# keikoproj/active-monitor

Measured on AMD Instinct MI355X. Metric: sustained_healthcheck_cycles_per_sec, higher is better.
Workload: dtype n/a; 1 GPU; model=healthcheck-controller, global_batch=1000, seq_len=0, parallelism=shard1x8w, crs_per_rank=1000, workers_per_rank=8, max_concurrent_crs=1000, cr_mix=49% repeatAfterSec, 30% cron, 20% failing-with-remedy, apiserver=http-subprocess-127.0.0.1

## Files before the change

active_monitor_amd/kube/http.py:

```python
from __future__ import annotations

import asyncio
import json
import logging
import re
import ssl
import time
from collections import deque
from typing import Any, AsyncIterator, Dict, List, Optional, Tuple
from urllib.parse import urlencode, urlsplit

import aiohttp

from ..utils import wirecodec
from .auth import Credential, CredentialSource
from .errors import (
    AlreadyExistsError,
    ApiError,
    BadRequestError,
    ConflictError,
    InvalidError,
    NotFoundError,
    UnauthorizedError,
)
# ... 233 lines not shown
    def __init__(self, qps: float, burst: int):
        self.qps = qps
        self.burst = float(burst)
        self.tokens = float(burst)
        self.last = time.monotonic()
        self._lock = asyncio.Lock()

    async def acquire(self) -> None:
        if self.qps <= 0:
            return
        async with self._lock:
            now = time.monotonic()
            self.tokens = min(self.burst, self.tokens + (now - self.last) * self.qps)
            self.last = now
            if self.tokens >= 1.0:
                self.tokens -= 1.0
                return
            wait = (1.0 - self.tokens) / self.qps
            self.tokens = 0.0
            await asyncio.sleep(wait)
            self.last = time.monotonic()


class _ConnPool:

    def __init__(self, host: str, port: int, max_conns: int = 32):
        self.host = host
        self.port = port
        self.max_conns = max_conns
        self._free: List[Tuple[asyncio.StreamReader, asyncio.StreamWriter]] = []
        self._count = 0
        self._waiters: "deque[asyncio.Future]" = deque()
        self._closed = False

    async def _acquire(self):
        while True:
            while self._free:
                reader, writer = self._free.pop()
                if writer.is_closing():
                    self._count -= 1
                    continue
                return reader, writer
            if self._count < self.max_conns:
                self._count += 1
                try:
                    return await asyncio.open_connection(self.host, self.port)
                except Exception:
                    self._count -= 1
                    raise
            fut = asyncio.get_running_loop().create_future()
            self._waiters.append(fut)
            await fut

    def _release(self, conn, reusable: bool) -> None:
        if reusable and not self._closed and not conn[1].is_closing():
            self._free.append(conn)
        else:
            self._count -= 1
            try:
                conn[1].close()
            except Exception:
                pass
        while self._waiters:
            fut = self._waiters.popleft()
            if not fut.done():
                fut.set_result(None)
                break

    async def request(self, method: str, target: str, headers: str,
                      body: Optional[bytes]) -> Tuple[int, bytes]:
        head = (
            f"{method} {target} HTTP/1.1\r\nHost: {self.host}:{self.port}\r\n"
            f"{headers}Content-Length: {len(body) if body else 0}\r\n\r\n"
        ).encode("latin-1")
        return await self._roundtrip(head + body if body else head)

    async def request_json(self, method: str, target: str, headers: str,
                           obj: Optional[Obj]) -> Tuple[int, bytes]:
        prefix = (
            f"{method} {target} HTTP/1.1\r\nHost: {self.host}:{self.port}\r\n"
            f"{headers}"
        ).encode("latin-1")
        return await self._roundtrip(wirecodec.frame(prefix, obj))

    async def _roundtrip(self, data: bytes) -> Tuple[int, bytes]:
        conn = await self._acquire()
        reader, writer = conn
        ok = False
        try:
            writer.write(data)
            await writer.drain()

            try:
                head = await reader.readuntil(b"\r\n\r\n")
            except asyncio.IncompleteReadError as e:
                if not e.partial:
                    raise ConnectionResetError("server closed connection") from None
                raise
            status, content_length, chunked, keep_alive = (
                wirecodec.parse_response_head(head)
            )
            if chunked:
                chunks = []
                while True:
                    size_line = await reader.readline()
                    size = int(size_line.strip().split(b";")[0], 16)
                    if size == 0:
                        await reader.readline()
                        break
                    chunks.append(await reader.readexactly(size))
                    await reader.readexactly(2)
                payload = b"".join(chunks)
            else:
                payload = await reader.readexactly(content_length) if content_length else b""
            ok = keep_alive
            return status, payload
        finally:
            self._release(conn, ok)

    def close(self) -> None:
        self._closed = True
        for _, writer in self._free:
            try:
                writer.close()
            except Exception:
                pass
        self._free.clear()
        while self._waiters:
            fut = self._waiters.popleft()
            if not fut.done():
                fut.set_exception(ConnectionError("connection pool closed"))


class HttpClient:
    def __init__(
        self,
        base_url: str,
        token: Optional[str] = None,
        verify: bool = True,
        ca_cert: Optional[str] = None,
        registry: Registry = DEFAULT_REGISTRY,
        qps: float = 20.0,
        burst: int = 30,
        credentials: Optional[CredentialSource] = None,
    ):
        self.base_url = base_url.rstrip("/")
        self.token = token
# ... 224 lines not shown
```

active_monitor_amd/kube/server.py:

```python
from __future__ import annotations

import asyncio
import hmac
import logging
from typing import List, Optional, Set, Tuple

from ..utils import wirecodec
from ..utils.wirecodec import EXPECT_CONTINUE, WANT_TABLE
from .errors import (
    ApiError,
    BadRequestError,
    ExpiredError,
    InvalidError,
    NotFoundError,
    UnauthorizedError,
)
from .memory import (
    MemoryApiServer,
    fields_match,
    labels_match,
    object_rv,
    parse_field_selector,
    parse_label_selector,
)
from .registry import WF_API_VERSION, WF_KIND

log = logging.getLogger("active_monitor_amd.kube.server")

_REASONS = {
    200: "OK", 201: "Created", 400: "Bad Request", 401: "Unauthorized",
    404: "Not Found",
# ... 75 lines not shown
        out = []
        for byte in path.encode("utf-8", "surrogatepass"):
            if byte in (0x22, 0x5C):
                out.append("\\" + chr(byte))
            elif 0x20 <= byte <= 0x7E and byte != 0x25:
                out.append(chr(byte))
            else:
                out.append(f"%{byte:02X}")
        return "".join(out)

    def prefix(self, status: int) -> bytes:
        lines = "".join(
            f'Warning: 299 - "unknown field \\"{self._header_text(p)}\\""\r\n'
            for p in self.paths
        )
        return _json_prefix(status) + lines.encode("ascii")


_OPEN_PATHS = frozenset({
    "/healthz", "/livez", "/readyz", "/version", "/version/",
})


class ApiServerFrontend:
    def __init__(self, server: MemoryApiServer, host: str = "127.0.0.1", port: int = 0,
                 accepted_tokens: Optional[Set[str]] = None, logs=None):
        self.server = server
        self.logs = logs
        self.host = host
        self.port = port
        self.accepted_tokens = accepted_tokens
        self.unauthorized_count = 0
        self._srv: Optional[asyncio.AbstractServer] = None
        self._live_subs: list = []

    @property
    def url(self) -> str:
        return f"http://{self.host}:{self.port}"

    async def start(self) -> None:
        self._srv = await asyncio.start_server(self._handle_conn, self.host, self.port)
        if self.port == 0:
            self.port = self._srv.sockets[0].getsockname()[1]

    async def stop(self) -> None:
        self.kick_watches()
        if self._srv is not None:
            self._srv.close()
            try:
                await asyncio.wait_for(self._srv.wait_closed(), 2.0)
            except asyncio.TimeoutError:
                pass

    def kick_watches(self) -> None:
        for sub in list(self._live_subs):
            sub.close()


    def _authorized(self, path: str, authorization: bytes) -> bool:
        if path in _OPEN_PATHS:
            return True
        ok = False
        scheme, _, presented = authorization.partition(b" ")
        if scheme.lower() == b"bearer":
            presented = presented.strip()
            for tok in list(self.accepted_tokens or ()):
                if hmac.compare_digest(presented, tok.encode("utf-8")):
                    ok = True
        if not ok:
            self.unauthorized_count += 1
        return ok

    @staticmethod
    def _unauthorized_response() -> bytes:
        return wirecodec.frame(
            _UNAUTHORIZED_PREFIX, _status_body(UnauthorizedError("Unauthorized"))
        )


    async def _handle_conn(self, reader: asyncio.StreamReader,
                           writer: asyncio.StreamWriter) -> None:
        try:
            while True:
                head = await reader.readuntil(b"\r\n\r\n")
                parsed = wirecodec.parse_request_head(head)
                if parsed is None:
                    return
                (method, path, query, content_length, content_type, flags,
                 authorization) = parsed
                if flags & EXPECT_CONTINUE:
                    writer.write(b"HTTP/1.1 100 Continue\r\n\r\n")
                    await writer.drain()
                body = await reader.readexactly(content_length) if content_length else b""

                if (self.accepted_tokens is not None
                        and not self._authorized(path, authorization)):
                    writer.write(self._unauthorized_response())
                    await writer.drain()
                    continue
                if query.get("watch") in ("true", "1"):
                    await self._serve_watch(writer, path, query)
                    return
                if path.endswith("/log") and self._is_log_route(path):
                    if await self._serve_log(writer, method, path, query):
                        return
                    continue
                status, obj = self._serve_unary(method, path, query, body,
                                                content_type)
                if (flags & WANT_TABLE and method == "GET" and status == 200
                        and isinstance(obj, dict)):
                    obj = self._to_table(obj)
                if type(obj) is dict or not isinstance(obj, (_Warned, str)):
                    writer.write(wirecodec.frame(_json_prefix(status), obj))
                elif isinstance(obj, _Warned):
                    writer.write(wirecodec.frame(obj.prefix(status), obj.obj))
                else:
                    payload = obj.encode()
                    writer.write(
                        (
                            f"HTTP/1.1 {status} {_REASONS.get(status, 'OK')}\r\n"
                            f"Content-Type: text/plain\r\n"
                            f"Content-Length: {len(payload)}\r\n\r\n"
                        ).encode("latin-1") + payload
                    )
                await writer.drain()
        except (ConnectionError, asyncio.IncompleteReadError,
                asyncio.LimitOverrunError, asyncio.CancelledError):
            pass
        except Exception:
            log.exception("frontend connection handler failed")
        finally:
            try:
                writer.close()
            except Exception:
                pass


    def _serve_unary(self, method: str, path: str, query: dict,
                     body: bytes, content_type: str = "") -> Tuple[int, Optional[dict]]:
        if path in ("/api", "/api/"):
            return 200, {"kind": "APIVersions", "versions": ["v1"]}
        if path in ("/apis", "/apis/"):
            return 200, self._discovery_apis()
        if path in ("/version", "/version/"):
            from .. import __version__

            return 200, {
                "major": "1", "minor": "33",
                "gitVersion": f"v1.33.0-active-monitor-amd+{__version__}",
            }
        if path in ("/healthz", "/readyz", "/livez"):
            return 200, "ok"
        route = _route(path)
        if route is None:
            return _failure(ApiError(f"the server could not find {path}"), 404)
        if not route[2]:
            return 200, self._resource_list(route[0])
        return self._dispatch(method, route, query, body, content_type)
# ... 195 lines not shown
                    "kind": "PartialObjectMetadata",
                    "apiVersion": "meta.k8s.io/v1",
                    "metadata": it.get("metadata", {}),
                },
            })
        return {
            "kind": "Table",
            "apiVersion": "meta.k8s.io/v1",
            "metadata": meta,
            "columnDefinitions": defs,
            "rows": rows,
        }


    def _is_log_route(self, path: str) -> bool:
        route = _route(path)
        if route is None or route[4] != "log" or route[0] != WF_API_VERSION:
            return False
        try:
            return self.server.registry.by_plural(route[0], route[2]).kind == WF_KIND
        except KeyError:
            return False

    async def _serve_log(self, writer: asyncio.StreamWriter, method: str,
                         path: str, query: dict) -> bool:
        _, namespace, _, name, _ = _route(path)
        try:
            if method != "GET":
                raise _MethodNotAllowed(f"unsupported method {method}")
            numbers = {}
            for key in ("tailLines", "limitBytes"):
                if query.get(key) is not None:
                    try:
                        numbers[key] = int(query[key])
                    except ValueError:
                        raise BadRequestError(
                            f"{key} must be an integer, not {query[key]!r}")
            self.server.get(WF_API_VERSION, WF_KIND, namespace, name)
            if self.logs is None:
                raise NotFoundError(
                    f"workflow {namespace}/{name} has no logs: this server "
                    "keeps no workflow logs")
            if not self.logs.has_run(namespace, name):
                raise NotFoundError(
                    f"workflow {namespace}/{name} has no logs: it was not run "
                    "by the local executor, or its logs were dropped for the "
                    "total size cap")
# ... 19 lines not shown
            return False
        self._live_subs.append(stream)
        try:
            writer.write(
                b"HTTP/1.1 200 OK\r\nContent-Type: text/plain\r\n"
                b"Transfer-Encoding: chunked\r\nConnection: close\r\n\r\n"
            )
            await writer.drain()
            async for chunk in stream:
                writer.write(b"%x\r\n%s\r\n" % (len(chunk), chunk))
                await writer.drain()
            writer.write(b"0\r\n\r\n")
            await writer.drain()
        except (ConnectionError, asyncio.CancelledError):
            pass
        finally:
            await stream.aclose()
            if stream in self._live_subs:
                self._live_subs.remove(stream)
        return True


    @staticmethod
    async def _refuse_watch(writer: asyncio.StreamWriter, err: ApiError,
                            status: int) -> None:
        status, body = _failure(err, status)
        writer.write(wirecodec.frame(_json_prefix(status), body))
        await writer.drain()

    async def _serve_watch(self, writer: asyncio.StreamWriter, path: str,
                           query: dict) -> None:
        route = _route(path)
        if route is None:
            return await self._refuse_watch(
                writer, ApiError(f"the server could not find {path}"), 404)
        api_version, namespace, plural = route[:3]
        namespace = namespace or None
        try:
            kind = self.server.registry.by_plural(api_version, plural).kind
        except KeyError:
            tail = [seg for seg in path.split("/") if seg][api_version.count("/") + 2:]
            return await self._refuse_watch(
                writer, ApiError("unknown resource " + "/".join(tail)), 404)

        rv_param = query.get("resourceVersion")
        selector: dict = {}
        fields: List[tuple] = []
        try:
            selector = parse_label_selector(query.get("labelSelector"))
        except ApiError:
            pass
        try:
            fields = parse_field_selector(query.get("fieldSelector"))
# ... 67 lines not shown
```

active_monitor_amd/utils/wirecodec.py:

```python
from __future__ import annotations

import json
import os
from typing import Any, Dict, Iterator, Optional, Tuple
from urllib.parse import parse_qsl, unquote, urlsplit

EXPECT_CONTINUE = 1
WANT_TABLE = 2

RequestHead = Tuple[str, str, Dict[str, str], int, str, int, bytes]
ResponseHead = Tuple[int, int, bool, bool]



def _py_dumpb(obj: Any) -> bytes:
    return json.dumps(obj, separators=(",", ":")).encode()


def _py_frame(prefix: bytes, obj: Any) -> bytes:
    payload = json.dumps(obj, separators=(",", ":")).encode() if obj is not None else b""
    return prefix + (
        f"Content-Length: {len(payload)}\r\n\r\n"
    ).encode("latin-1") + payload

# ... 55 lines not shown

def _py_parse_response_head(head: bytes) -> ResponseHead:
    lines = _head_lines(head)
    status_line = next(lines, b"")
    if not status_line:
        raise ConnectionResetError("server closed connection")
    status = int(status_line.split(b" ", 2)[1])
    content_length = 0
    chunked = False
    keep_alive = True
    for line in lines:
        if line in (b"\r\n", b"\n", b""):
            break
        lower = line.lower()
        if lower.startswith(b"content-length:"):
            content_length = int(line.split(b":", 1)[1])
        elif lower.startswith(b"transfer-encoding:") and b"chunked" in lower:
            chunked = True
        elif lower.startswith(b"connection:") and b"close" in lower:
            keep_alive = False
    return status, content_length, chunked, keep_alive



try:
    from active_monitor_amd import _amcore

    _json_dumpb = _amcore.json_dumpb
    _json_frame = _amcore.json_frame
    _json_loadb = _amcore.json_loadb
    _parse_request_head = _amcore.parse_request_head
    _parse_response_head = _amcore.parse_response_head
    HAVE_NATIVE = True
except (ImportError, AttributeError):
    if os.environ.get("AM_REQUIRE_NATIVE") == "1":
        raise ImportError(
            "the native wire codec in active_monitor_amd._amcore is required "
            "(AM_REQUIRE_NATIVE=1) but not built; run "
            "`python setup.py build_ext --inplace`"
        )
    HAVE_NATIVE = False

if HAVE_NATIVE:
    def _native_dumpb(obj: Any) -> bytes:
        out = _json_dumpb(obj)
        if out is NotImplemented:
            return _py_dumpb(obj)
        return out

    def _native_frame(prefix: bytes, obj: Any) -> bytes:
        out = _json_frame(prefix, obj)
        if out is NotImplemented:
            return _py_frame(prefix, obj)
        return out

# ... 18 lines not shown
    def _native_parse_response_head(head: bytes) -> ResponseHead:
        out = _parse_response_head(head)
        if out is NotImplemented:
            return _py_parse_response_head(head)
        return out


NATIVE = HAVE_NATIVE and os.environ.get("AM_WIRE_NATIVE") != "0"

if NATIVE:
    dumpb = _native_dumpb
    frame = _native_frame
    loads_strict = _native_loads_strict
    loads_lenient = _native_loads_lenient
    parse_request_head = _native_parse_request_head
    parse_response_head = _native_parse_response_head
else:
    dumpb = _py_dumpb
    frame = _py_frame
    loads_strict = _py_loads_strict
    loads_lenient = _py_loads_lenient
    parse_request_head = _py_parse_request_head
    parse_response_head = _py_parse_response_head
```

native/_amcore.c:

```c
#define PY_SSIZE_T_CLEAN
#include <Python.h>

#include "wirehead.h"
#include "wirejson.h"

static PyObject *copy_deepcopy = NULL;

static PyObject *am_deep_copy_obj(PyObject *obj);

static PyObject *
am_copy_dict(PyObject *obj)
{
    PyObject *out = PyDict_New();
    if (out == NULL)
        return NULL;
    Py_ssize_t pos = 0;
    PyObject *key, *value;
    while (PyDict_Next(obj, &pos, &key, &value)) {
        PyObject *cv = am_deep_copy_obj(value);
        if (cv == NULL) {
            Py_DECREF(out);
            return NULL;
        }
        if (PyDict_SetItem(out, key, cv) < 0) {
            Py_DECREF(cv);
// ... 97 lines not shown
            continue;
        }
        PyObject *cv = am_deep_copy_obj(value);
        if (cv == NULL || PyDict_SetItem(out, key, cv) < 0) {
            Py_XDECREF(cv);
            Py_DECREF(key);
            Py_DECREF(out);
            return NULL;
        }
        Py_DECREF(cv);
        Py_DECREF(key);
    }
    return out;
}


static PyObject *
span_str(am_span s)
{
    return PyUnicode_FromStringAndSize(s.p, (Py_ssize_t)s.n);
}

static PyObject *
am_py_parse_request_head(PyObject *self, PyObject *head)
{
    (void)self;
    Py_buffer view;
    if (PyObject_GetBuffer(head, &view, PyBUF_SIMPLE) < 0)
        return NULL;
    am_request_head h;
    PyObject *out = NULL, *query = NULL;
    if (am_parse_request_head(view.buf, (size_t)view.len, &h) != AM_HEAD_OK) {
        out = Py_NotImplemented;
        Py_INCREF(out);
        goto done;
    }
    query = PyDict_New();
    if (query == NULL)
        goto done;
    size_t pos = 0;
    am_span name, value;
    while (am_query_next(h.query.p, h.query.n, &pos, &name, &value)) {
        PyObject *k = span_str(name), *v = span_str(value);
        int rc = (k && v) ? PyDict_SetItem(query, k, v) : -1;
        Py_XDECREF(k);
        Py_XDECREF(v);
        if (rc < 0)
            goto done;
    }
    out = Py_BuildValue("(s#s#OLs#iy#)",
                        h.method.p, (Py_ssize_t)h.method.n,
                        h.path.p, (Py_ssize_t)h.path.n,
                        query, h.content_length,
                        h.content_type.p, (Py_ssize_t)h.content_type.n,
                        h.flags,
                        h.authorization.p, (Py_ssize_t)h.authorization.n);
done:
    Py_XDECREF(query);
    PyBuffer_Release(&view);
    return out;
}

static PyObject *
am_py_parse_response_head(PyObject *self, PyObject *head)
{
    (void)self;
    Py_buffer view;
    if (PyObject_GetBuffer(head, &view, PyBUF_SIMPLE) < 0)
        return NULL;
    am_response_head h;
    int rc = am_parse_response_head(view.buf, (size_t)view.len, &h);
    PyBuffer_Release(&view);
    if (rc != AM_HEAD_OK)
        Py_RETURN_NOTIMPLEMENTED;
    return Py_BuildValue("(iLOO)", h.status, h.content_length,
                         h.chunked ? Py_True : Py_False,
                         h.keep_alive ? Py_True : Py_False);
}

static PyMethodDef am_methods[] = {
    {"deep_copy", am_deep_copy, METH_O,
     "Fast deep copy of a JSON-shaped object tree."},
    {"snapshot", am_snapshot, METH_O,
     "Read-optimized object copy: private metadata/status, shared spec."},
    {"json_dumpb", am_json_dumpb, METH_O,
     "Compact JSON bytes of a JSON-shaped tree, or NotImplemented."},
    {"json_frame", (PyCFunction)(void (*)(void))am_json_frame, METH_FASTCALL,
     "prefix + Content-Length line + JSON payload as one bytes, or "
     "NotImplemented."},
    {"json_loadb", am_json_loadb, METH_O,
     "Parse UTF-8 JSON from a bytes-like object, or NotImplemented."},
    {"parse_request_head", am_py_parse_request_head, METH_O,
     "(method, path, query, content_length, content_type, flags, "
     "authorization) of one complete request head, or NotImplemented."},
    {"parse_response_head", am_py_parse_response_head, METH_O,
     "(status, content_length, chunked, keep_alive) of one complete "
     "response head, or NotImplemented."},
    {NULL, NULL, 0, NULL},
};

static struct PyModuleDef am_module = {
    PyModuleDef_HEAD_INIT, "_amcore",
    "Native hot-path primitives for active-monitor-amd.", -1, am_methods,
    NULL, NULL, NULL, NULL,
};

PyMODINIT_FUNC
PyInit__amcore(void)
{
    PyObject *copy_mod = PyImport_ImportModule("copy");
    if (copy_mod == NULL)
        return NULL;
    copy_deepcopy = PyObject_GetAttrString(copy_mod, "deepcopy");
    Py_DECREF(copy_mod);
    if (copy_deepcopy == NULL)
        return NULL;
    return PyModule_Create(&am_module);
}
```

setup.py:

```python
import os

from setuptools import Extension, setup
from setuptools.command.build_ext import build_ext


class OptionalBuildExt(build_ext):

    def run(self):
        try:
            super().run()
        except Exception as e:
            print(f"warning: skipping native extension build: {e}")

    def build_extension(self, ext):
        try:
            super().build_extension(ext)
        except Exception as e:
            print(f"warning: skipping {ext.name}: {e}")


setup(
    ext_modules=[
        Extension(
            "active_monitor_amd._amcore",
            sources=[os.path.join("native", name) for name in
                     ("_amcore.c", "wirejson.c", "wirehead.c")],
            depends=[os.path.join("native", name) for name in
                     ("wirejson.h", "wirehead.h")],
            extra_compile_args=["-O2"],
        )
    ],
    cmdclass={"build_ext": OptionalBuildExt},
)
```

Before: 3968 healthcheck cycles/s.

## Replace asyncio streams with protocol-based HTTP client and server using native framer

Both the HTTP client connection pool and the API server frontend move from asyncio StreamReader/StreamWriter coroutines to asyncio.Protocol callbacks. A new native C framer splits incoming bytes into complete request or response messages, falling back to Python when it cannot handle a message. Unary requests are answered synchronously inside data_received, and watch and log routes still run as tasks with reading paused. The intent is to cut per-request coroutine, await and stream-buffer overhead on the loopback apiserver path. In exchange it adds subtle flow-control, pipelining and error-handling logic that must reproduce the old stream semantics.

```diff
diff --git a/active_monitor_amd/kube/http.py b/active_monitor_amd/kube/http.py
--- a/active_monitor_amd/kube/http.py
+++ b/active_monitor_amd/kube/http.py
@@ -279,43 +279,112 @@
             self.last = time.monotonic()
 
 
+class _Conn(asyncio.Protocol):
+
+    __slots__ = ("transport", "waiter", "framer", "feed", "partial",
+                 "reusable", "lost")
+
+    def __init__(self) -> None:
+        self.transport: Any = None
+        self.waiter: Optional[asyncio.Future] = None
+        self.framer = wirecodec.framer("response")
+        self.feed = self.framer.feed
+        self.partial = False
+        self.reusable = True
+        self.lost = False
+
+    def connection_made(self, transport) -> None:
+        self.transport = transport
+
+    def data_received(self, data: bytes) -> None:
+        waiter = self.waiter
+        if waiter is None or waiter.done():
+            self.reusable = False
+            self.transport.close()
+            return
+        try:
+            messages = self.feed(data)
+            framer = self.framer
+            if framer.bailed:
+                self.framer, more = wirecodec.continue_in_python(framer, "response")
+                self.feed = self.framer.feed
+                messages += more
+                framer = self.framer
+            if framer.error:
+                raise asyncio.LimitOverrunError(
+                    "response head exceeds the length limit", framer.buffered)
+        except Exception as e:
+            self.waiter = None
+            self.reusable = False
+            waiter.set_exception(e)
+            self.transport.close()
+            return
+        if not messages:
+            self.partial = True
+            return
+        if len(messages) > 1 or framer.buffered:
+            self.reusable = False
+        self.waiter = None
+        self.partial = False
+        waiter.set_result(messages[0])
+
+    def connection_lost(self, exc: Optional[Exception]) -> None:
+        self.lost = True
+        self.reusable = False
+        waiter, self.waiter = self.waiter, None
+        if waiter is None or waiter.done():
+            return
+        if self.partial:
+            err: Exception = asyncio.IncompleteReadError(self.framer.pending(), None)
+        else:
+            err = ConnectionResetError("server closed connection")
+        err.__cause__ = exc
+        waiter.set_exception(err)
+
+    def is_closing(self) -> bool:
+        return self.lost or self.transport.is_closing()
+
+
 class _ConnPool:
 
     def __init__(self, host: str, port: int, max_conns: int = 32):
         self.host = host
         self.port = port
         self.max_conns = max_conns
-        self._free: List[Tuple[asyncio.StreamReader, asyncio.StreamWriter]] = []
+        self._free: List[_Conn] = []
         self._count = 0
         self._waiters: "deque[asyncio.Future]" = deque()
         self._closed = False
 
-    async def _acquire(self):
+    async def _acquire(self) -> _Conn:
         while True:
             while self._free:
-                reader, writer = self._free.pop()
-                if writer.is_closing():
+                conn = self._free.pop()
+                if conn.is_closing():
                     self._count -= 1
                     continue
-                return reader, writer
+                return conn
+            loop = asyncio.get_running_loop()
             if self._count < self.max_conns:
                 self._count += 1
                 try:
-                    return await asyncio.open_connection(self.host, self.port)
-                except Exception:
+                    _, conn = await loop.create_connection(
+                        _Conn, self.host, self.port)
+                    return conn
+                except BaseException:
                     self._count -= 1
                     raise
-            fut = asyncio.get_running_loop().create_future()
+            fut = loop.create_future()
             self._waiters.append(fut)
             await fut
 
-    def _release(self, conn, reusable: bool) -> None:
-        if reusable and not self._closed and not conn[1].is_closing():
+    def _release(self, conn: _Conn, reusable: bool) -> None:
+        if reusable and not self._closed and not conn.is_closing():
             self._free.append(conn)
         else:
             self._count -= 1
             try:
-                conn[1].close()
+                conn.transport.close()
             except Exception:
                 pass
         while self._waiters:
@@ -341,45 +410,26 @@
         return await self._roundtrip(wirecodec.frame(prefix, obj))
 
     async def _roundtrip(self, data: bytes) -> Tuple[int, bytes]:
-        conn = await self._acquire()
-        reader, writer = conn
-        ok = False
+        free = self._free
+        if free and not free[-1].is_closing():
+            conn = free.pop()
+        else:
+            conn = await self._acquire()
+        waiter = conn.waiter = asyncio.get_running_loop().create_future()
         try:
-            writer.write(data)
-            await writer.drain()
-
-            try:
-                head = await reader.readuntil(b"\r\n\r\n")
-            except asyncio.IncompleteReadError as e:
-                if not e.partial:
-                    raise ConnectionResetError("server closed connection") from None
-                raise
-            status, content_length, chunked, keep_alive = (
-                wirecodec.parse_response_head(head)
-            )
-            if chunked:
-                chunks = []
-                while True:
-                    size_line = await reader.readline()
-                    size = int(size_line.strip().split(b";")[0], 16)
-                    if size == 0:
-                        await reader.readline()
-                        break
-                    chunks.append(await reader.readexactly(size))
-                    await reader.readexactly(2)
-                payload = b"".join(chunks)
-            else:
-                payload = await reader.readexactly(content_length) if content_length else b""
-            ok = keep_alive
-            return status, payload
-        finally:
-            self._release(conn, ok)
+            conn.transport.write(data)
+            status, keep_alive, payload = await waiter
+        except BaseException:
+            self._release(conn, False)
+            raise
+        self._release(conn, keep_alive and conn.reusable)
+        return status, payload
 
     def close(self) -> None:
         self._closed = True
-        for _, writer in self._free:
+        for conn in self._free:
             try:
-                writer.close()
+                conn.transport.close()
             except Exception:
                 pass
         self._free.clear()
diff --git a/active_monitor_amd/kube/server.py b/active_monitor_amd/kube/server.py
--- a/active_monitor_amd/kube/server.py
+++ b/active_monitor_amd/kube/server.py
@@ -3,10 +3,10 @@
 import asyncio
 import hmac
 import logging
-from typing import List, Optional, Set, Tuple
+from typing import Any, List, Optional, Set, Tuple
 
 from ..utils import wirecodec
-from ..utils.wirecodec import EXPECT_CONTINUE, WANT_TABLE
+from ..utils.wirecodec import WANT_TABLE
 from .errors import (
     ApiError,
     BadRequestError,
@@ -128,6 +128,153 @@
 })
 
 
+class _TaskWriter:
+
+    __slots__ = ("_conn",)
+
+    def __init__(self, conn: "_FrontendConn"):
+        self._conn = conn
+
+    def write(self, data: bytes) -> None:
+        self._conn.transport.write(data)
+
+    async def drain(self) -> None:
+        conn = self._conn
+        if conn.transport.is_closing() and not conn.lost:
+            await asyncio.sleep(0)
+        if conn.lost:
+            raise ConnectionResetError("Connection lost")
+        if conn.write_paused:
+            waiter = asyncio.get_running_loop().create_future()
+            conn.drain_waiters.append(waiter)
+            await waiter
+
+    def close(self) -> None:
+        self._conn.transport.close()
+
+    def is_closing(self) -> bool:
+        return self._conn.lost or self._conn.transport.is_closing()
+
+
+class _FrontendConn(asyncio.Protocol):
+
+    __slots__ = ("frontend", "transport", "framer", "feed", "task", "backlog",
+                 "write_paused", "drain_waiters", "lost")
+
+    def __init__(self, frontend: "ApiServerFrontend"):
+        self.frontend = frontend
+        self.transport: Any = None
+        self.framer = wirecodec.framer("request")
+        self.feed = self.framer.feed
+        self.task: Optional[asyncio.Task] = None
+        self.backlog: list = []
+        self.write_paused = False
+        self.drain_waiters: list = []
+        self.lost = False
+
+    def connection_made(self, transport) -> None:
+        self.transport = transport
+        self.frontend._conns.add(self)
+
+    def connection_lost(self, exc: Optional[Exception]) -> None:
+        self.lost = True
+        self.frontend._conns.discard(self)
+        self.backlog.clear()
+        for waiter in self.drain_waiters:
+            if not waiter.done():
+                waiter.set_exception(ConnectionResetError("Connection lost"))
+        self.drain_waiters.clear()
+        if self.task is not None:
+            self.task.cancel()
+
+    def pause_writing(self) -> None:
+        self.write_paused = True
+        self.transport.pause_reading()
+
+    def resume_writing(self) -> None:
+        self.write_paused = False
+        for waiter in self.drain_waiters:
+            if not waiter.done():
+                waiter.set_result(None)
+        self.drain_waiters.clear()
+        if self.task is None:
+            self._resume()
+
+    def data_received(self, data: bytes) -> None:
+        try:
+            messages = self.feed(data)
+            framer = self.framer
+            if framer.bailed:
+                self.framer, more = wirecodec.continue_in_python(framer, "request")
+                self.feed = self.framer.feed
+                messages += more
+                framer = self.framer
+            if self.backlog:
+                self.backlog += messages
+            elif messages:
+                self._serve(messages)
+            if framer.error:
+                self.transport.close()
+            elif framer.expect_pending:
+                framer.expect_pending = False
+                self.transport.write(b"HTTP/1.1 100 Continue\r\n\r\n")
+        except Exception:
+            log.exception("frontend connection handler failed")
+            self.transport.close()
+
+    def _serve(self, messages: list) -> None:
+        frontend = self.frontend
+        write = self.transport.write
+        for i, message in enumerate(messages):
+            if self.task is not None or self.write_paused or self.lost:
+                self.backlog += messages[i:]
+                return
+            (method, path, query, _, content_type, flags, authorization,
+             body) = message
+            if (frontend.accepted_tokens is not None
+                    and not frontend._authorized(path, authorization)):
+                write(frontend._unauthorized_response())
+            elif query.get("watch") in ("true", "1"):
+                self._start(frontend._serve_watch(_TaskWriter(self), path, query),
+                            owns=True)
+            elif path.endswith("/log") and frontend._is_log_route(path):
+                self._start(frontend._serve_log(_TaskWriter(self), method, path,
+                                                query), owns=False)
+            else:
+                write(frontend._unary_response(method, path, query, body,
+                                               content_type, flags))
+
+    def _start(self, coro, owns: bool) -> None:
+        self.transport.pause_reading()
+        self.task = asyncio.ensure_future(self._run(coro, owns))
+
+    async def _run(self, coro, owns: bool) -> None:
+        try:
+            owns = bool(await coro) or owns
+        except (ConnectionError, asyncio.CancelledError):
+            owns = True
+        except Exception:
+            log.exception("frontend connection handler failed")
+            owns = True
+        finally:
+            self.task = None
+        if owns or self.lost:
+            self.transport.close()
+        else:
+            self._resume()
+
+    def _resume(self) -> None:
+        try:
+            if self.backlog:
+                messages, self.backlog = self.backlog, []
+                self._serve(messages)
+            if self.task is None and not self.write_paused and not self.lost:
+                self.transport.resume_reading()
+        except Exception:
+            log.exception("frontend connection handler failed")
+            self.transport.close()
+
+
 class ApiServerFrontend:
     def __init__(self, server: MemoryApiServer, host: str = "127.0.0.1", port: int = 0,
                  accepted_tokens: Optional[Set[str]] = None, logs=None):
@@ -139,13 +286,15 @@
         self.unauthorized_count = 0
         self._srv: Optional[asyncio.AbstractServer] = None
         self._live_subs: list = []
+        self._conns: Set["_FrontendConn"] = set()
 
     @property
     def url(self) -> str:
         return f"http://{self.host}:{self.port}"
 
     async def start(self) -> None:
-        self._srv = await asyncio.start_server(self._handle_conn, self.host, self.port)
+        self._srv = await asyncio.get_running_loop().create_server(
+            lambda: _FrontendConn(self), self.host, self.port)
         if self.port == 0:
             self.port = self._srv.sockets[0].getsockname()[1]
 
@@ -184,62 +333,22 @@
         )
 
 
-    async def _handle_conn(self, reader: asyncio.StreamReader,
-                           writer: asyncio.StreamWriter) -> None:
-        try:
-            while True:
-                head = await reader.readuntil(b"\r\n\r\n")
-                parsed = wirecodec.parse_request_head(head)
-                if parsed is None:
-                    return
-                (method, path, query, content_length, content_type, flags,
-                 authorization) = parsed
-                if flags & EXPECT_CONTINUE:
-                    writer.write(b"HTTP/1.1 100 Continue\r\n\r\n")
-                    await writer.drain()
-                body = await reader.readexactly(content_length) if content_length else b""
-
-                if (self.accepted_tokens is not None
-                        and not self._authorized(path, authorization)):
-                    writer.write(self._unauthorized_response())
-                    await writer.drain()
-                    continue
-                if query.get("watch") in ("true", "1"):
-                    await self._serve_watch(writer, path, query)
-                    return
-                if path.endswith("/log") and self._is_log_route(path):
-                    if await self._serve_log(writer, method, path, query):
-                        return
-                    continue
-                status, obj = self._serve_unary(method, path, query, body,
-                                                content_type)
-                if (flags & WANT_TABLE and method == "GET" and status == 200
-                        and isinstance(obj, dict)):
-                    obj = self._to_table(obj)
-                if type(obj) is dict or not isinstance(obj, (_Warned, str)):
-                    writer.write(wirecodec.frame(_json_prefix(status), obj))
-                elif isinstance(obj, _Warned):
-                    writer.write(wirecodec.frame(obj.prefix(status), obj.obj))
-                else:
-                    payload = obj.encode()
-                    writer.write(
-                        (
-                            f"HTTP/1.1 {status} {_REASONS.get(status, 'OK')}\r\n"
-                            f"Content-Type: text/plain\r\n"
-                            f"Content-Length: {len(payload)}\r\n\r\n"
-                        ).encode("latin-1") + payload
-                    )
-                await writer.drain()
-        except (ConnectionError, asyncio.IncompleteReadError,
-                asyncio.LimitOverrunError, asyncio.CancelledError):
-            pass
-        except Exception:
-            log.exception("frontend connection handler failed")
-        finally:
-            try:
-                writer.close()
-            except Exception:
-                pass
+    def _unary_response(self, method: str, path: str, query: dict, body: bytes,
+                        content_type: str, flags: int) -> bytes:
+        status, obj = self._serve_unary(method, path, query, body, content_type)
+        if (flags & WANT_TABLE and method == "GET" and status == 200
+                and isinstance(obj, dict)):
+            obj = self._to_table(obj)
+        if type(obj) is dict or not isinstance(obj, (_Warned, str)):
+            return wirecodec.frame(_json_prefix(status), obj)
+        if isinstance(obj, _Warned):
+            return wirecodec.frame(obj.prefix(status), obj.obj)
+        payload = obj.encode()
+        return (
+            f"HTTP/1.1 {status} {_REASONS.get(status, 'OK')}\r\n"
+            f"Content-Type: text/plain\r\n"
+            f"Content-Length: {len(payload)}\r\n\r\n"
+        ).encode("latin-1") + payload
 
 
     def _serve_unary(self, method: str, path: str, query: dict,
@@ -481,7 +590,7 @@
         except KeyError:
             return False
 
-    async def _serve_log(self, writer: asyncio.StreamWriter, method: str,
+    async def _serve_log(self, writer: _TaskWriter, method: str,
                          path: str, query: dict) -> bool:
         _, namespace, _, name, _ = _route(path)
         try:
@@ -547,13 +656,13 @@
 
 
     @staticmethod
-    async def _refuse_watch(writer: asyncio.StreamWriter, err: ApiError,
+    async def _refuse_watch(writer: _TaskWriter, err: ApiError,
                             status: int) -> None:
         status, body = _failure(err, status)
         writer.write(wirecodec.frame(_json_prefix(status), body))
         await writer.drain()
 
-    async def _serve_watch(self, writer: asyncio.StreamWriter, path: str,
+    async def _serve_watch(self, writer: _TaskWriter, path: str,
                            query: dict) -> None:
         route = _route(path)
         if route is None:
diff --git a/active_monitor_amd/utils/wirecodec.py b/active_monitor_amd/utils/wirecodec.py
--- a/active_monitor_amd/utils/wirecodec.py
+++ b/active_monitor_amd/utils/wirecodec.py
@@ -101,6 +101,137 @@
     return status, content_length, chunked, keep_alive
 
 
+HEAD_LIMIT = 65536
+_TERM = b"\r\n\r\n"
+_HEAD, _BODY, _CHUNK_SIZE, _CHUNK_DATA, _CHUNK_TRAILER = range(5)
+
+
+class PyFramer:
+
+    bailed = False
+
+    def __init__(self, kind: str, seed: bytes = b""):
+        if kind not in ("request", "response"):
+            raise ValueError("kind must be 'request' or 'response'")
+        self._request = kind == "request"
+        self._buf = bytearray(seed)
+        self._state = _HEAD
+        self._scan = 0
+        self._head: Any = None
+        self._need = 0
+        self._chunks: list = []
+        self.error = False
+        self.expect_pending = False
+
+    @property
+    def buffered(self) -> int:
+        return len(self._buf)
+
+    def pending(self) -> bytes:
+        return bytes(self._buf)
+
+    def feed(self, data: bytes = b"") -> list:
+        out: list = []
+        if self.error:
+            return out
+        buf = self._buf
+        if data:
+            buf += data
+        pos = 0
+        try:
+            while True:
+                state = self._state
+                avail = len(buf) - pos
+                if state == _HEAD:
+                    isep = buf.find(_TERM, pos + self._scan)
+                    if isep < 0:
+                        earliest = avail
+                        for k in (3, 2, 1):
+                            if avail >= k and buf.endswith(_TERM[:k]):
+                                earliest = avail - k
+                                break
+                        if earliest >= HEAD_LIMIT:
+                            self.error = True
+                        self._scan = max(0, avail - 3)
+                        break
+                    if isep - pos >= HEAD_LIMIT:
+                        self.error = True
+                        break
+                    head = bytes(buf[pos:isep + 4])
+                    if self._request:
+                        parsed = _py_parse_request_head(head)
+                        if parsed is None:
+                            self.error = True
+                            break
+                        self._head = parsed
+                        self._need = parsed[3]
+                        self._state = _BODY
+                        if (parsed[5] & EXPECT_CONTINUE
+                                and len(buf) - isep - 4 < self._need):
+                            self.expect_pending = True
+                    else:
+                        status, length, chunked, keep_alive = (
+                            _py_parse_response_head(head))
+                        self._head = (status, keep_alive)
+                        if chunked:
+                            self._chunks = []
+                            self._state = _CHUNK_SIZE
+                        else:
+                            self._need = length
+                            self._state = _BODY
+                    if self._need < 0:
+                        raise ValueError("negative Content-Length")
+                    pos = isep + 4
+                    self._scan = 0
+                elif state == _BODY:
+                    need = self._need
+                    if avail < need:
+                        break
+                    body = bytes(buf[pos:pos + need])
+                    pos += need
+                    out.append(self._head + (body,))
+                    self._state = _HEAD
+                elif state == _CHUNK_DATA:
+                    need = self._need
+                    if avail < need + 2:
+                        break
+                    self._chunks.append(bytes(buf[pos:pos + need]))
+                    pos += need + 2
+                    self._state = _CHUNK_SIZE
+                else:
+                    nl = buf.find(b"\n", pos + self._scan)
+                    if nl < 0:
+                        if avail >= HEAD_LIMIT:
+                            self.error = True
+                        self._scan = avail
+                        break
+                    line = bytes(buf[pos:nl + 1])
+                    pos = nl + 1
+                    self._scan = 0
+                    if state == _CHUNK_TRAILER:
+                        out.append(self._head + (b"".join(self._chunks),))
+                        self._chunks = []
+                        self._state = _HEAD
+                        continue
+                    size = int(line.strip().split(b";")[0], 16)
+                    if size == 0:
+                        self._state = _CHUNK_TRAILER
+                    elif size < 0:
+                        raise ValueError("negative chunk size")
+                    else:
+                        self._need = size
+                        self._state = _CHUNK_DATA
+        finally:
+            if pos:
+                del buf[:pos]
+        return out
+
+
+def continue_in_python(native_framer: Any, kind: str) -> Tuple["PyFramer", list]:
+    framer = PyFramer(kind, native_framer.pending())
+    return framer, framer.feed()
+
+
 
 try:
     from active_monitor_amd import _amcore
@@ -110,6 +241,7 @@
     _json_loadb = _amcore.json_loadb
     _parse_request_head = _amcore.parse_request_head
     _parse_response_head = _amcore.parse_response_head
+    _Framer = _amcore.Framer
     HAVE_NATIVE = True
 except (ImportError, AttributeError):
     if os.environ.get("AM_REQUIRE_NATIVE") == "1":
@@ -174,3 +306,7 @@
     loads_lenient = _py_loads_lenient
     parse_request_head = _py_parse_request_head
     parse_response_head = _py_parse_response_head
+
+
+def framer(kind: str) -> Any:
+    return _Framer(kind) if NATIVE else PyFramer(kind)
diff --git a/native/_amcore.c b/native/_amcore.c
--- a/native/_amcore.c
+++ b/native/_amcore.c
@@ -1,6 +1,7 @@
 #define PY_SSIZE_T_CLEAN
 #include <Python.h>
 
+#include "wireframe.h"
 #include "wirehead.h"
 #include "wirejson.h"
 
@@ -144,25 +145,15 @@
 }
 
 static PyObject *
-am_py_parse_request_head(PyObject *self, PyObject *head)
-{
-    (void)self;
-    Py_buffer view;
-    if (PyObject_GetBuffer(head, &view, PyBUF_SIMPLE) < 0)
-        return NULL;
-    am_request_head h;
-    PyObject *out = NULL, *query = NULL;
-    if (am_parse_request_head(view.buf, (size_t)view.len, &h) != AM_HEAD_OK) {
-        out = Py_NotImplemented;
-        Py_INCREF(out);
-        goto done;
-    }
-    query = PyDict_New();
+request_tuple(const am_request_head *h, const am_span *body)
+{
+    PyObject *out = NULL;
+    PyObject *query = PyDict_New();
     if (query == NULL)
-        goto done;
+        return NULL;
     size_t pos = 0;
     am_span name, value;
-    while (am_query_next(h.query.p, h.query.n, &pos, &name, &value)) {
+    while (am_query_next(h->query.p, h->query.n, &pos, &name, &value)) {
         PyObject *k = span_str(name), *v = span_str(value);
         int rc = (k && v) ? PyDict_SetItem(query, k, v) : -1;
         Py_XDECREF(k);
@@ -170,15 +161,43 @@
         if (rc < 0)
             goto done;
     }
-    out = Py_BuildValue("(s#s#OLs#iy#)",
-                        h.method.p, (Py_ssize_t)h.method.n,
-                        h.path.p, (Py_ssize_t)h.path.n,
-                        query, h.content_length,
-                        h.content_type.p, (Py_ssize_t)h.content_type.n,
-                        h.flags,
-                        h.authorization.p, (Py_ssize_t)h.authorization.n);
+    if (body == NULL)
+        out = Py_BuildValue("(s#s#OLs#iy#)",
+                            h->method.p, (Py_ssize_t)h->method.n,
+                            h->path.p, (Py_ssize_t)h->path.n,
+                            query, h->content_length,
+                            h->content_type.p, (Py_ssize_t)h->content_type.n,
+                            h->flags,
+                            h->authorization.p, (Py_ssize_t)h->authorization.n);
+    else
+        out = Py_BuildValue("(s#s#OLs#iy#y#)",
+                            h->method.p, (Py_ssize_t)h->method.n,
+                            h->path.p, (Py_ssize_t)h->path.n,
+                            query, h->content_length,
+                            h->content_type.p, (Py_ssize_t)h->content_type.n,
+                            h->flags,
+                            h->authorization.p, (Py_ssize_t)h->authorization.n,
+                            body->p, (Py_ssize_t)body->n);
 done:
-    Py_XDECREF(query);
+    Py_DECREF(query);
+    return out;
+}
+
+static PyObject *
+am_py_parse_request_head(PyObject *self, PyObject *head)
+{
+    (void)self;
+    Py_buffer view;
+    if (PyObject_GetBuffer(head, &view, PyBUF_SIMPLE) < 0)
+        return NULL;
+    am_request_head h;
+    PyObject *out;
+    if (am_parse_request_head(view.buf, (size_t)view.len, &h) != AM_HEAD_OK) {
+        out = Py_NotImplemented;
+        Py_INCREF(out);
+    } else {
+        out = request_tuple(&h, NULL);
+    }
     PyBuffer_Release(&view);
     return out;
 }
@@ -199,6 +218,154 @@
                          h.chunked ? Py_True : Py_False,
                          h.keep_alive ? Py_True : Py_False);
 }
+
+
+typedef struct {
+    PyObject_HEAD
+    am_framer f;
+} FramerObject;
+
+static int
+Framer_init(FramerObject *self, PyObject *args, PyObject *kwds)
+{
+    static char *names[] = {"kind", NULL};
+    const char *kind;
+    if (!PyArg_ParseTupleAndKeywords(args, kwds, "s:Framer", names, &kind))
+        return -1;
+    int k;
+    if (strcmp(kind, "request") == 0)
+        k = AM_FRAME_REQUEST;
+    else if (strcmp(kind, "response") == 0)
+        k = AM_FRAME_RESPONSE;
+    else {
+        PyErr_SetString(PyExc_ValueError,
+                        "kind must be 'request' or 'response'");
+        return -1;
+    }
+    am_framer_free(&self->f);
+    am_framer_init(&self->f, k);
+    return 0;
+}
+
+static void
+Framer_dealloc(FramerObject *self)
+{
+    am_framer_free(&self->f);
+    Py_TYPE(self)->tp_free((PyObject *)self);
+}
+
+static PyObject *
+Framer_feed(FramerObject *self, PyObject *data)
+{
+    Py_buffer view;
+    if (PyObject_GetBuffer(data, &view, PyBUF_SIMPLE) < 0)
+        return NULL;
+    PyObject *out = PyList_New(0);
+    if (out == NULL)
+        goto fail;
+    if (am_framer_feed(&self->f, view.buf, (size_t)view.len) < 0) {
+        PyErr_NoMemory();
+        goto fail;
+    }
+    am_message m;
+    while (am_framer_next(&self->f, &m) == AM_FRAME_MESSAGE) {
+        PyObject *msg;
+        if (self->f.kind == AM_FRAME_REQUEST)
+            msg = request_tuple(&m.h.request, &m.body);
+        else
+            msg = Py_BuildValue("(iOy#)", m.h.response.status,
+                                m.h.response.keep_alive ? Py_True : Py_False,
+                                m.body.p, (Py_ssize_t)m.body.n);
+        int rc = msg ? PyList_Append(out, msg) : -1;
+        Py_XDECREF(msg);
+        if (rc < 0) {
+            am_framer_end(&self->f);
+            self->f.state = AM_FRAME_ERROR;
+            goto fail;
+        }
+    }
+    if (am_framer_end(&self->f) < 0) {
+        PyErr_NoMemory();
+        goto fail;
+    }
+    PyBuffer_Release(&view);
+    return out;
+fail:
+    Py_XDECREF(out);
+    PyBuffer_Release(&view);
+    return NULL;
+}
+
+static PyObject *
+Framer_pending(FramerObject *self, PyObject *noargs)
+{
+    (void)noargs;
+    return PyBytes_FromStringAndSize(self->f.len ? self->f.buf : "",
+                                     (Py_ssize_t)self->f.len);
+}
+
+static PyObject *
+Framer_get_bailed(FramerObject *self, void *closure)
+{
+    (void)closure;
+    return PyBool_FromLong(self->f.state == AM_FRAME_BAIL);
+}
+
+static PyObject *
+Framer_get_error(FramerObject *self, void *closure)
+{
+    (void)closure;
+    return PyBool_FromLong(self->f.state == AM_FRAME_ERROR);
+}
+
+static PyObject *
+Framer_get_buffered(FramerObject *self, void *closure)
+{
+    (void)closure;
+    return PyLong_FromSize_t(self->f.len);
+}
+
+static PyObject *
+Framer_get_false(FramerObject *self, void *closure)
+{
+    (void)self;
+    (void)closure;
+    Py_RETURN_FALSE;
+}
+
+static PyMethodDef Framer_methods[] = {
+    {"feed", (PyCFunction)Framer_feed, METH_O,
+     "Add the bytes of one read; the list of messages they complete."},
+    {"pending", (PyCFunction)Framer_pending, METH_NOARGS,
+     "The bytes fed but not yet part of a returned message."},
+    {NULL, NULL, 0, NULL},
+};
+
+static PyGetSetDef Framer_getset[] = {
+    {"bailed", (getter)Framer_get_bailed, NULL,
+     "True once a message needs the Python framer.", NULL},
+    {"error", (getter)Framer_get_error, NULL,
+     "True once a head passed the length limit without its terminator.", NULL},
+    {"buffered", (getter)Framer_get_buffered, NULL,
+     "len(pending()).", NULL},
+    {"expect_pending", (getter)Framer_get_false, NULL,
+     "Always False: a request with an Expect flag bails.", NULL},
+    {NULL, NULL, NULL, NULL, NULL},
+};
+
+static PyTypeObject FramerType = {
+    PyVarObject_HEAD_INIT(NULL, 0)
+    .tp_name = "_amcore.Framer",
+    .tp_doc = "Framer(kind): incremental HTTP/1.1 message framer; kind is "
+              "'request' or 'response'.",
+    .tp_basicsize = sizeof(FramerObject),
+    .tp_flags = Py_TPFLAGS_DEFAULT,
+    .tp_new = PyType_GenericNew,
+    .tp_init = (initproc)Framer_init,
+    .tp_dealloc = (destructor)Framer_dealloc,
+    .tp_methods = Framer_methods,
+    .tp_getset = Framer_getset,
+};
 
 static PyMethodDef am_methods[] = {
     {"deep_copy", am_deep_copy, METH_O,
@@ -237,5 +404,16 @@
     Py_DECREF(copy_mod);
     if (copy_deepcopy == NULL)
         return NULL;
-    return PyModule_Create(&am_module);
-}
+    if (PyType_Ready(&FramerType) < 0)
+        return NULL;
+    PyObject *mod = PyModule_Create(&am_module);
+    if (mod == NULL)
+        return NULL;
+    Py_INCREF(&FramerType);
+    if (PyModule_AddObject(mod, "Framer", (PyObject *)&FramerType) < 0) {
+        Py_DECREF(&FramerType);
+        Py_DECREF(mod);
+        return NULL;
+    }
+    return mod;
+}
diff --git a/native/check/check_frame.c b/native/check/check_frame.c
--- /dev/null
+++ b/native/check/check_frame.c
@@ -0,0 +1,280 @@
+#include "wireframe.h"
+
+#include <stdio.h>
+#include <stdlib.h>
+#include <string.h>
+
+#define BIG 70000
+
+static unsigned long feeds;
+
+static void
+die(const char *what, size_t at)
+{
+    fprintf(stderr, "check_frame: %s (at %zu)\n", what, at);
+    exit(1);
+}
+
+typedef struct {
+    char *p;
+    size_t n;
+} text;
+
+static void
+add(text *t, const char *s, size_t n)
+{
+    t->p = realloc(t->p, t->n + n + 1);
+    if (t->p == NULL)
+        abort();
+    memcpy(t->p + t->n, s, n);
+    t->n += n;
+}
+
+static void
+adds(text *t, const char *s)
+{
+    add(t, s, strlen(s));
+}
+
+static void
+add_big(text *t)
+{
+    char *b = malloc(BIG);
+    if (b == NULL)
+        abort();
+    for (size_t i = 0; i < BIG; i++)
+        b[i] = (char)(i < 69888 ? i & 0xff : 'x');
+    add(t, b, BIG);
+    free(b);
+}
+
+typedef struct {
+    size_t messages;
+    size_t body_bytes;
+    unsigned long long sum;
+} tally;
+
+static void
+mix(tally *t, const char *p, size_t n)
+{
+    for (size_t i = 0; i < n; i++) {
+        t->sum ^= (unsigned char)p[i];
+        t->sum *= 1099511628211ULL;
+    }
+}
+
+static int
+feed(am_framer *f, const char *data, size_t n, tally *t)
+{
+    char *chunk = malloc(n ? n : 1);
+    if (chunk == NULL)
+        abort();
+    memcpy(chunk, data, n);
+    if (am_framer_feed(f, chunk, n) != 0)
+        die("feed: out of memory", n);
+    am_message m;
+    int rc;
+    while ((rc = am_framer_next(f, &m)) == AM_FRAME_MESSAGE) {
+        const char *lo = f->win, *hi = f->win + f->win_len;
+        if (m.head.p < lo || m.head.p + m.head.n != m.body.p
+                || m.body.p + m.body.n > hi)
+            die("message outside its window", n);
+        if (m.head.n < 4 || memcmp(m.body.p - 4, "\r\n\r\n", 4) != 0)
+            die("head does not end at the terminator", n);
+        if (f->kind == AM_FRAME_REQUEST) {
+            if ((size_t)m.h.request.content_length != m.body.n
+                    || m.h.request.method.p < m.head.p
+                    || m.h.request.path.p + m.h.request.path.n > m.body.p)
+                die("request fields", n);
+        } else if ((size_t)m.h.response.content_length != m.body.n) {
+            die("response fields", n);
+        }
+        t->messages++;
+        t->body_bytes += m.body.n;
+        mix(t, m.head.p, m.head.n);
+        mix(t, m.body.p, m.body.n);
+    }
+    if (rc != AM_FRAME_MORE && rc != AM_FRAME_BAIL && rc != AM_FRAME_ERROR)
+        die("bad result of am_framer_next", n);
+    if (am_framer_end(f) != 0)
+        die("end: out of memory", n);
+    free(chunk);
+    feeds++;
+    return rc;
+}
+
+static tally
+start(void)
+{
+    tally t = {0, 0, 14695981039346656037ULL};
+    return t;
+}
+
+static void
+same(const tally *a, const tally *b, const char *what, size_t at)
+{
+    if (a->messages != b->messages || a->body_bytes != b->body_bytes
+            || a->sum != b->sum)
+        die(what, at);
+}
+
+static void
+corpus(int kind, const text *data, size_t messages, size_t tail)
+{
+    am_framer f;
+    tally whole = start();
+    am_framer_init(&f, kind);
+    if (feed(&f, data->p, data->n, &whole) != AM_FRAME_MORE)
+        die("corpus did not end in MORE", 0);
+    if (whole.messages != messages || f.len != tail
+            || memcmp(f.buf, data->p + data->n - tail, tail) != 0)
+        die("corpus fed whole: wrong messages or rest", whole.messages);
+    am_framer_free(&f);
+
+    tally bytes = start();
+    am_framer_init(&f, kind);
+    for (size_t i = 0; i < data->n; i++)
+        feed(&f, data->p + i, 1, &bytes);
+    same(&whole, &bytes, "byte by byte differs from whole", 0);
+    if (f.len != tail)
+        die("byte by byte: wrong rest", f.len);
+    am_framer_free(&f);
+
+    for (size_t i = 0; i <= data->n; i++) {
+        tally cut = start();
+        am_framer_init(&f, kind);
+        feed(&f, data->p, i, &cut);
+        feed(&f, data->p + i, data->n - i, &cut);
+        same(&whole, &cut, "a split differs from whole", i);
+        if (f.len != tail || f.state != AM_FRAME_MORE
+                || memcmp(f.buf, data->p + data->n - tail, tail) != 0)
+            die("a split: wrong rest", i);
+        am_framer_free(&f);
+    }
+}
+
+static void
+bail(int kind, const char *good, const char *bad)
+{
+    text data = {NULL, 0};
+    adds(&data, good);
+    adds(&data, bad);
+    adds(&data, good);
+    size_t rest = strlen(bad) + strlen(good);
+    for (size_t i = 0; i <= data.n; i++) {
+        am_framer f;
+        tally t = start();
+        am_framer_init(&f, kind);
+        feed(&f, data.p, i, &t);
+        int rc = feed(&f, data.p + i, data.n - i, &t);
+        if (rc != AM_FRAME_BAIL || f.state != AM_FRAME_BAIL || t.messages != 1)
+            die("no bail after one message", i);
+        if (f.len != rest || memcmp(f.buf, data.p + data.n - rest, rest) != 0)
+            die("bail: pending is not the unconsumed suffix", i);
+        if (feed(&f, "more", 4, &t) != AM_FRAME_BAIL || f.len != rest + 4
+                || memcmp(f.buf + rest, "more", 4) != 0 || t.messages != 1)
+            die("bail: bytes fed afterwards are not kept", i);
+        am_framer_free(&f);
+    }
+    free(data.p);
+}
+
+static void
+head_limit(int kind)
+{
+    const char *first = kind == AM_FRAME_REQUEST
+        ? "GET /x HTTP/1.1\r\nX-Pad: " : "HTTP/1.1 200 OK\r\nX-Pad: ";
+    text data = {NULL, 0};
+    adds(&data, first);
+    while (data.n < AM_HEAD_LIMIT)
+        add(&data, "a", 1);
+    am_framer f;
+    tally t = start();
+
+    text ok = {NULL, 0};
+    add(&ok, data.p, AM_HEAD_LIMIT - 1);
+    adds(&ok, "\r\n\r\n");
+    am_framer_init(&f, kind);
+    if (feed(&f, ok.p, ok.n, &t) != AM_FRAME_MORE || t.messages != 1)
+        die("a head of 65,535 bytes was refused", 0);
+    am_framer_free(&f);
+    am_framer_init(&f, kind);
+    for (size_t i = 0; i < ok.n; i++)
+        if (feed(&f, ok.p + i, 1, &t) != AM_FRAME_MORE)
+            die("a head of 65,535 bytes was refused in bytes", i);
+    if (t.messages != 2)
+        die("a head of 65,535 bytes in bytes gave no message", 0);
+    am_framer_free(&f);
+
+    am_framer_init(&f, kind);
+    if (feed(&f, data.p, AM_HEAD_LIMIT - 1, &t) != AM_FRAME_MORE)
+        die("error before the limit", 0);
+    if (feed(&f, data.p + AM_HEAD_LIMIT - 1, 1, &t) != AM_FRAME_ERROR)
+        die("no error at the limit", 0);
+    if (feed(&f, "\r\n\r\n", 4, &t) != AM_FRAME_ERROR || f.len != 0)
+        die("the error state does not last", 0);
+    am_framer_free(&f);
+    free(ok.p);
+    free(data.p);
+}
+
+int
+main(void)
+{
+    text rq = {NULL, 0};
+    adds(&rq, "GET /apis/activemonitor.keikoproj.io/v1alpha1/namespaces/health/healthchecks"
+              "?labelSelector=a=b&limit=500&empty= HTTP/1.1\r\nHost: 127.0.0.1:1\r\n"
+              "Content-Type: application/json\r\nAuthorization:  Bearer s3cr3t \r\n"
+              "Content-Length: 0\r\n\r\n"
+              "POST /api/v1/namespaces/health/configmaps HTTP/1.1\r\ncontent-length: 1\r\n\r\n7"
+              "PUT /x HTTP/1.1\r\nContent-Type: application/json\r\n"
+              "Content-Length: 70000\r\n\r\n");
+    add_big(&rq);
+    adds(&rq, "GET /api/v1/pods HTTP/1.1\r\nAccept: application/json;as=Table;v=v1\r\n\r\n"
+              "DELETE /y HTTP/1.1\r\n\r\n");
+    const char *rq_tail = "GET /half HTTP/1.1\r\nHost: h\r\nContent-Le";
+    adds(&rq, rq_tail);
+    corpus(AM_FRAME_REQUEST, &rq, 5, strlen(rq_tail));
+    free(rq.p);
+
+    text rs = {NULL, 0};
+    adds(&rs, "HTTP/1.1 200 OK\r\nContent-Type: application/json\r\nContent-Length: 0\r\n\r\n"
+              "HTTP/1.1 201 Created\r\nContent-Length: 1\r\n\r\n{"
+              "HTTP/1.1 200 OK\r\nContent-Length: 70000\r\n\r\n");
+    add_big(&rs);
+    adds(&rs, "HTTP/1.1 404 Not Found\r\nConnection: close\r\nContent-Length: 17\r\n\r\n"
+              "{\"kind\":\"Status\"}"
+              "HTTP/1.1 204\r\n\r\n");
+    const char *rs_tail = "HTTP/1.1 200 OK\r\nContent-Length: 5\r\n\r\nhal";
+    adds(&rs, rs_tail);
+    corpus(AM_FRAME_RESPONSE, &rs, 5, strlen(rs_tail));
+    free(rs.p);
+
+    const char *good_rq = "GET /ok HTTP/1.1\r\nHost: h\r\n\r\n";
+    const char *good_rs = "HTTP/1.1 200 OK\r\nContent-Length: 2\r\n\r\nok";
+    bail(AM_FRAME_REQUEST, good_rq,
+         "PUT /x HTTP/1.1\r\nHost: h\nX-Y: z\r\nContent-Length: 2\r\n\r\nok");
+    bail(AM_FRAME_REQUEST, good_rq, "GET /a%20b?x=1%2B1 HTTP/1.1\r\nHost: h\r\n\r\n");
+    bail(AM_FRAME_REQUEST, good_rq,
+         "POST /big HTTP/1.1\r\nExpect: 100-continue\r\nContent-Length: 4\r\n\r\nbody");
+    bail(AM_FRAME_RESPONSE, good_rs,
+         "HTTP/1.1 200 OK\r\nTransfer-Encoding: chunked\r\n\r\n"
+         "5\r\nhello\r\n6;ext=1\r\n world\r\n0\r\n\r\n");
+    bail(AM_FRAME_RESPONSE, good_rs,
+         "HTTP/1.1 200 OK\r\nContent-Length: 9999999999999999999\r\n\r\n");
+
+    head_limit(AM_FRAME_REQUEST);
+    head_limit(AM_FRAME_RESPONSE);
+
+    am_framer f;
+    tally t = start();
+    am_framer_init(&f, AM_FRAME_RESPONSE);
+    const char *huge = "HTTP/1.1 200 OK\r\nContent-Length: 999999999999999999\r\n\r\nabc";
+    if (feed(&f, huge, strlen(huge), &t) != AM_FRAME_MORE || f.len != strlen(huge)
+            || f.cap > 4096)
+        die("a huge Content-Length did not just wait", f.cap);
+    am_framer_free(&f);
+
+    printf("check_frame: %lu feeds, no report\n", feeds);
+    return 0;
+}
diff --git a/native/wireframe.c b/native/wireframe.c
--- /dev/null
+++ b/native/wireframe.c
@@ -0,0 +1,170 @@
+#include "wireframe.h"
+
+#include <stdlib.h>
+#include <string.h>
+
+static const char TERM[4] = {'\r', '\n', '\r', '\n'};
+
+void
+am_framer_init(am_framer *f, int kind)
+{
+    memset(f, 0, sizeof(*f));
+    f->kind = kind;
+    f->state = AM_FRAME_MORE;
+}
+
+void
+am_framer_free(am_framer *f)
+{
+    free(f->buf);
+    f->buf = NULL;
+    f->len = f->cap = 0;
+}
+
+static int
+reserve(am_framer *f, size_t need)
+{
+    if (need <= f->cap)
+        return 0;
+    size_t cap = f->cap ? f->cap : 4096;
+    while (cap < need) {
+        if (cap > ((size_t)-1) / 2)
+            return AM_FRAME_NOMEM;
+        cap *= 2;
+    }
+    char *p = realloc(f->buf, cap);
+    if (p == NULL)
+        return AM_FRAME_NOMEM;
+    f->buf = p;
+    f->cap = cap;
+    return 0;
+}
+
+static size_t
+find_term(const char *p, size_t n)
+{
+    size_t i = 0;
+    while (n - i >= 4) {
+        const char *cr = memchr(p + i, '\r', n - i - 3);
+        if (cr == NULL)
+            break;
+        i = (size_t)(cr - p);
+        if (memcmp(cr, TERM, 4) == 0)
+            return i;
+        i++;
+    }
+    return n;
+}
+
+int
+am_framer_feed(am_framer *f, const char *data, size_t len)
+{
+    if (f->in_feed)
+        am_framer_end(f);
+    if (f->state == AM_FRAME_ERROR)
+        len = 0;
+    if (f->len == 0 && f->state == AM_FRAME_MORE) {
+        f->win = data;
+        f->win_len = len;
+        f->borrowed = 1;
+    } else {
+        if (len > ((size_t)-1) - f->len || reserve(f, f->len + len) < 0)
+            return AM_FRAME_NOMEM;
+        if (len)
+            memcpy(f->buf + f->len, data, len);
+        f->len += len;
+        f->win = f->buf;
+        f->win_len = f->len;
+        f->borrowed = 0;
+    }
+    f->off = 0;
+    f->in_feed = 1;
+    return 0;
+}
+
+int
+am_framer_next(am_framer *f, am_message *out)
+{
+    if (f->state != AM_FRAME_MORE || !f->in_feed)
+        return f->state;
+    const char *p = f->win + f->off;
+    size_t avail = f->win_len - f->off;
+    size_t scan = f->scan < avail ? f->scan : avail;
+    size_t isep = scan + find_term(p + scan, avail - scan);
+    if (isep == avail) {
+        size_t earliest = avail;
+        for (size_t k = 3; k >= 1; k--) {
+            if (avail >= k && memcmp(p + avail - k, TERM, k) == 0) {
+                earliest = avail - k;
+                break;
+            }
+        }
+        if (earliest >= AM_HEAD_LIMIT)
+            return f->state = AM_FRAME_ERROR;
+        f->scan = avail > 3 ? avail - 3 : 0;
+        return AM_FRAME_MORE;
+    }
+    if (isep >= AM_HEAD_LIMIT)
+        return f->state = AM_FRAME_ERROR;
+
+    size_t head_len = isep + 4;
+    long long content_length;
+    if (f->kind == AM_FRAME_REQUEST) {
+        if (am_parse_request_head(p, head_len, &out->h.request) != AM_HEAD_OK
+                || (out->h.request.flags & AM_FLAG_EXPECT_CONTINUE))
+            return f->state = AM_FRAME_BAIL;
+        content_length = out->h.request.content_length;
+    } else {
+        if (am_parse_response_head(p, head_len, &out->h.response) != AM_HEAD_OK
+                || out->h.response.chunked)
+            return f->state = AM_FRAME_BAIL;
+        content_length = out->h.response.content_length;
+    }
+    if (content_length < 0)
+        return f->state = AM_FRAME_BAIL;
+    if ((unsigned long long)content_length > avail - head_len) {
+        f->scan = isep;
+        return AM_FRAME_MORE;
+    }
+    out->head.p = p;
+    out->head.n = head_len;
+    out->body.p = p + head_len;
+    out->body.n = (size_t)content_length;
+    f->off += head_len + (size_t)content_length;
+    f->scan = 0;
+    return AM_FRAME_MESSAGE;
+}
+
+int
+am_framer_end(am_framer *f)
+{
+    if (!f->in_feed)
+        return 0;
+    size_t rest = f->win_len - f->off;
+    int rc = 0;
+    if (f->state == AM_FRAME_ERROR) {
+        rest = 0;
+    } else if (f->borrowed) {
+        if (rest > 0) {
+            if (reserve(f, rest) < 0) {
+                f->state = AM_FRAME_ERROR;
+                rest = 0;
+                rc = AM_FRAME_NOMEM;
+            } else {
+                memcpy(f->buf, f->win + f->off, rest);
+            }
+        }
+    } else if (f->off > 0 && rest > 0) {
+        memmove(f->buf, f->buf + f->off, rest);
+    }
+    f->len = rest;
+    if (rest == 0 && f->cap > (1u << 20)) {
+        free(f->buf);
+        f->buf = NULL;
+        f->cap = 0;
+    }
+    f->win = NULL;
+    f->win_len = f->off = 0;
+    f->in_feed = 0;
+    return rc;
+}
diff --git a/native/wireframe.h b/native/wireframe.h
--- /dev/null
+++ b/native/wireframe.h
@@ -0,0 +1,49 @@
+#ifndef AM_WIREFRAME_H
+#define AM_WIREFRAME_H
+
+#include <stddef.h>
+
+#include "wirehead.h"
+
+#define AM_FRAME_REQUEST 0
+#define AM_FRAME_RESPONSE 1
+
+#define AM_FRAME_MORE 0
+#define AM_FRAME_MESSAGE 1
+#define AM_FRAME_BAIL 2
+#define AM_FRAME_ERROR 3
+
+#define AM_FRAME_NOMEM (-1)
+
+#define AM_HEAD_LIMIT 65536
+
+typedef struct {
+    int kind;
+    int state;
+    char *buf;
+    size_t len, cap;
+    const char *win;
+    size_t win_len;
+    size_t off;
+    size_t scan;
+    int in_feed;
+    int borrowed;
+} am_framer;
+
+typedef struct {
+    am_span head;
+    am_span body;
+    union {
+        am_request_head request;
+        am_response_head response;
+    } h;
+} am_message;
+
+void am_framer_init(am_framer *f, int kind);
+void am_framer_free(am_framer *f);
+
+int am_framer_feed(am_framer *f, const char *data, size_t len);
+int am_framer_next(am_framer *f, am_message *out);
+int am_framer_end(am_framer *f);
+
+#endif
diff --git a/setup.py b/setup.py
--- a/setup.py
+++ b/setup.py
@@ -24,9 +24,9 @@
         Extension(
             "active_monitor_amd._amcore",
             sources=[os.path.join("native", name) for name in
-                     ("_amcore.c", "wirejson.c", "wirehead.c")],
+                     ("_amcore.c", "wirejson.c", "wirehead.c", "wireframe.c")],
             depends=[os.path.join("native", name) for name in
-                     ("wirejson.h", "wirehead.h")],
+                     ("wirejson.h", "wirehead.h", "wireframe.h")],
             extra_compile_args=["-O2"],
         )
     ],
```

New measurement: 4343 healthcheck cycles/s, median of 5. 1.09x the previous value.
